# krocki/Eigen-LSTM

Measured on AMD Instinct MI355X. Metric: chars/sec fwd+BPTT, enwik6 H=512 S=100 B=64, 1/2/4/8 GPU, higher is better.
Workload: dtype f32; 1 GPU; configs[2] (headline): enwik6.txt, hidden=512 seq=100 batch=64, fp32; run as hidden=512 seq=100 batch=64/GPU (global 64), fp32, enwik6-sized synthetic text (1000000 bytes), stride-1 windows from a full window, Adagrad lr=0.01; parallelism=single, engine=default, gemm=native

## Files before the change

eigen-lstm_amd/csrc/persistent.hip:

```cpp
#include <type_traits>
#include "kernels.h"
#include "../../include/lstm_hip.h"

#include <cstdlib>

namespace lstmk {

typedef float f32x4 __attribute__((ext_vector_type(4)));
typedef unsigned int u32x4 __attribute__((ext_vector_type(4)));

#pragma clang fp contract(off)
__device__ __forceinline__ float p_exp_neg(float x) {
    const float hi = 1.44269502162933349609375f, lo = 1.925963033500011e-08f;
    const float t = -x * hi;
    const float r = __builtin_fmaf(-x, hi, -t) - x * lo;
    return __builtin_amdgcn_exp2f(t) * (1.0f + r * 0.693147180559945f);
}
template <bool FAST> __device__ __forceinline__ float p_sigm(float x) {
    if (FAST) return __frcp_rn(1.0f + __expf(-x));
    return __builtin_amdgcn_rcpf(1.0f + p_exp_neg(x));
}
template <bool FAST> __device__ __forceinline__ float p_tanh(float x) {
    if (FAST) return 1.0f - 2.0f * __frcp_rn(__expf(2.0f * x) + 1.0f);
    const float e = p_exp_neg(2.0f * __builtin_fabsf(x));
    return __builtin_copysignf((1.0f - e) * __builtin_amdgcn_rcpf(1.0f + e), x);
}

__device__ __forceinline__ float xchg_row16(float v, int l) {
    const unsigned x = __builtin_bit_cast(unsigned, v);
    const auto r = __builtin_amdgcn_permlane16_swap(x, x, false, false);
    return __builtin_bit_cast(float, (l & 16) ? r[0] : r[1]);
}
__device__ __forceinline__ float xchg_half32(float v, int l) {
    const unsigned x = __builtin_bit_cast(unsigned, v);
    const auto r = __builtin_amdgcn_permlane32_swap(x, x, false, false);
    return __builtin_bit_cast(float, (l & 32) ? r[0] : r[1]);
}

template <int CTRL> __device__ __forceinline__ float dpp_f(float v) {
    return __builtin_bit_cast(float, __builtin_amdgcn_update_dpp(0, __builtin_bit_cast(int, v), CTRL, 0xf, 0xf, false));
}

#ifndef XCD_LOCAL
#define XCD_LOCAL 1
#endif
#ifndef XCD_FORCE_LOCAL
#define XCD_FORCE_LOCAL 0
#endif
#ifndef BWD_PF
#define BWD_PF 6
#endif
#ifndef FWD_PF
#define FWD_PF 4
#endif

#ifndef CNT_STRIDE_U
#define CNT_STRIDE_U 16
#endif
constexpr int CNT_STRIDE = CNT_STRIDE_U;
#ifndef GROUP_REMAP
#define GROUP_REMAP 1
#endif
#ifndef FWD_SH
#define FWD_SH 64
#endif
#ifndef BWD_SH
#define BWD_SH 8
#endif
constexpr int CNT_SLOTS = 64;
constexpr int SPIN_LIMIT = 1 << 21;

__device__ __forceinline__ __amdgpu_buffer_rsrc_t make_rsrc(const void *p, size_t bytes) {
    const unsigned n = bytes > 0x7ffffff0ull ? 0x7ffffff0u : (unsigned)bytes;
    return __builtin_amdgcn_make_buffer_rsrc(const_cast<void *>(p), 0, (int)n, 0x00020000);
}
__device__ __forceinline__ float4 ld_sc1(__amdgpu_buffer_rsrc_t r, int byte_off) {
    const u32x4 v = __builtin_amdgcn_raw_buffer_load_b128(r, byte_off, 0, 16);
    float4 f;
    f.x = __uint_as_float(v.x);
    f.y = __uint_as_float(v.y);
    f.z = __uint_as_float(v.z);
    f.w = __uint_as_float(v.w);
    return f;
}
__device__ __forceinline__ void st_sc1(float4 f, __amdgpu_buffer_rsrc_t r, int byte_off) {
    u32x4 v;
    v.x = __float_as_uint(f.x);
    v.y = __float_as_uint(f.y);
    v.z = __float_as_uint(f.z);
    v.w = __float_as_uint(f.w);
    __builtin_amdgcn_raw_buffer_store_b128(v, r, byte_off, 0, 16);
}

#ifndef POLL_SLEEP
#define POLL_SLEEP 1
#endif
template <int CNT_SH>
__device__ __forceinline__ bool wait_arrivals(const unsigned *cp, int n_prod, unsigned epoch, unsigned *abortp, int lane) {
    const unsigned expect = lane < CNT_SH ? epoch * (unsigned)((n_prod - lane + CNT_SH - 1) / CNT_SH) : 0u;
    for (int spins = 0;; spins++) {
        unsigned v = 0;
        if (lane < CNT_SH) v = __hip_atomic_load(cp + lane * CNT_STRIDE, __ATOMIC_RELAXED, __HIP_MEMORY_SCOPE_AGENT);
        if (__all(v >= expect)) return true;
        if (spins > SPIN_LIMIT) break;
        if ((spins & 255) == 255 && __hip_atomic_load(abortp, __ATOMIC_RELAXED, __HIP_MEMORY_SCOPE_AGENT) != 0) break;
        __builtin_amdgcn_s_sleep(POLL_SLEEP);
    }
    if (lane == 0) __hip_atomic_store(abortp, 1u, __ATOMIC_RELAXED, __HIP_MEMORY_SCOPE_AGENT);
    return false;
}

template <int NK4W, bool FAST>
__global__ __launch_bounds__(256) void k_fwd_persistent(const float4 *__restrict__ Ufwd, const float *__restrict__ W,
                                                        const float *__restrict__ bias, float *H, float *__restrict__ C,
                                                        float *__restrict__ G, const int32_t *__restrict__ xi,
                                                        unsigned *cnt, unsigned *abortp, unsigned epoch, int S, int B) {
    constexpr int N = 64 * NK4W, G4 = 4 * N, nk4 = N / 16;
    __shared__ float red[4 * 4 * 64];
    __shared__ int s_abort;
    const int l = threadIdx.x & 63, w = threadIdx.x >> 6;
    const int NB = gridDim.x, NG = gridDim.y;
    const int lin_ = blockIdx.x + NB * blockIdx.y;
    const int p = GROUP_REMAP ? lin_ / NG : (int)blockIdx.x, g = GROUP_REMAP ? lin_ % NG : (int)blockIdx.y;
    const int q = l >> 4, c = l & 15;
    const int col = 16 * g + c, colc = col < B ? col : B - 1;
    const int j = 4 * p + q;

    float4 a[NK4W];
#pragma unroll
    for (int i = 0; i < NK4W; i++) a[i] = Ufwd[((size_t)p * nk4 + w * NK4W + i) * 64 + l];
    float bs[4] = {0.f, 0.f, 0.f, 0.f}, cprev = 0.f;
    if (w == 0) {
#pragma unroll
        for (int gt = 0; gt < 4; gt++) bs[gt] = bias[gt * N + j];
        cprev = C[(size_t)colc * N + j];
    }
    const __amdgpu_buffer_rsrc_t rH = make_rsrc(H, (size_t)S * N * B * sizeof(float));
    if (threadIdx.x == 0) s_abort = 0;
    __syncthreads();
    for (int t = 1; t < S; t++) {
        float wx[4] = {0.f, 0.f, 0.f, 0.f};
        if (w == 0) {
            const int x = xi[t * B + colc];
            if (x >= 0) {
#pragma unroll
                for (int gt = 0; gt < 4; gt++) wx[gt] = W[(size_t)x * G4 + gt * N + j];
            }
            if (t > 1) {
                const unsigned *cp = cnt + (size_t)((t - 1) * NG + g) * CNT_SLOTS * CNT_STRIDE;
                if (!wait_arrivals<FWD_SH>(cp, NB, epoch, abortp, l) && l == 0) s_abort = 1;
            }
        }
        __syncthreads();
        if (s_abort) return;

        const int off = (int)((((size_t)(t - 1) * B + colc) * N + 16 * (w * NK4W) + 4 * q) * sizeof(float));
        constexpr int PF = FWD_PF < NK4W ? FWD_PF : NK4W;
        float4 b[NK4W];
#pragma unroll
        for (int i = 0; i < PF; i++) b[i] = ld_sc1(rH, off + 64 * i);
        __builtin_amdgcn_sched_barrier(0);
        f32x4 acc0 = {0.f, 0.f, 0.f, 0.f}, acc1 = {0.f, 0.f, 0.f, 0.f};
#pragma unroll
        for (int i = 0; i < NK4W; i++) {
            if (i + PF < NK4W) b[i + PF] = ld_sc1(rH, off + 64 * (i + PF));
            if (i & 1) {
                acc1 = __builtin_amdgcn_mfma_f32_16x16x4f32(a[i].x, b[i].x, acc1, 0, 0, 0);
                acc1 = __builtin_amdgcn_mfma_f32_16x16x4f32(a[i].y, b[i].y, acc1, 0, 0, 0);
                acc1 = __builtin_amdgcn_mfma_f32_16x16x4f32(a[i].z, b[i].z, acc1, 0, 0, 0);
                acc1 = __builtin_amdgcn_mfma_f32_16x16x4f32(a[i].w, b[i].w, acc1, 0, 0, 0);
            } else {
                acc0 = __builtin_amdgcn_mfma_f32_16x16x4f32(a[i].x, b[i].x, acc0, 0, 0, 0);
                acc0 = __builtin_amdgcn_mfma_f32_16x16x4f32(a[i].y, b[i].y, acc0, 0, 0, 0);
                acc0 = __builtin_amdgcn_mfma_f32_16x16x4f32(a[i].z, b[i].z, acc0, 0, 0, 0);
                acc0 = __builtin_amdgcn_mfma_f32_16x16x4f32(a[i].w, b[i].w, acc0, 0, 0, 0);
            }
            __builtin_amdgcn_sched_barrier(0);
        }
#pragma unroll
        for (int r = 0; r < 4; r++) red[(w * 4 + r) * 64 + l] = acc0[r] + acc1[r];
        __syncthreads();

        if (w == 0) {
            float pre[4];
#pragma unroll
            for (int gt = 0; gt < 4; gt++) {
                const float uh = ((red[(0 * 4 + gt) * 64 + l] + red[(1 * 4 + gt) * 64 + l]) + red[(2 * 4 + gt) * 64 + l]) +
                                 red[(3 * 4 + gt) * 64 + l];
                pre[gt] = (wx[gt] + uh) + bs[gt];
            }
            const float ig = p_sigm<FAST>(pre[0]), og = p_sigm<FAST>(pre[1]), fg = p_sigm<FAST>(pre[2]);
            const float ug = p_tanh<FAST>(pre[3]);
            const float cv = p_tanh<FAST>(ig * ug + fg * cprev);
            const float hv = og * cv;
            cprev = cv;
            float4 h4;
            h4.x = __shfl(hv, c, 64);
            h4.y = __shfl(hv, 16 + c, 64);
            h4.z = __shfl(hv, 32 + c, 64);
            h4.w = __shfl(hv, 48 + c, 64);
                if (q == 0 && col < B) st_sc1(h4, rH, (int)((((size_t)t * B + col) * N + 4 * p) * sizeof(float)));
            if (t + 1 < S) {
                asm volatile("s_waitcnt vmcnt(0)" ::: "memory");
                        if (l == 0)
                    __hip_atomic_fetch_add(cnt + ((size_t)(t * NG + g) * CNT_SLOTS + (p & (FWD_SH - 1))) * CNT_STRIDE, 1u, __ATOMIC_RELAXED,
                                           __HIP_MEMORY_SCOPE_AGENT);
            }
            if (col < B) {
                float *gc = G + ((size_t)t * B + col) * G4 + j;
                gc[0] = ig;
                gc[N] = og;
                gc[2 * N] = fg;
                gc[3 * N] = ug;
                C[((size_t)t * B + col) * N + j] = cv;
            }
        }
    }
}

template <int NKW, bool FAST>
__global__ __launch_bounds__(512) void k_fwd_persistent2(const float4 *__restrict__ Ufwd, const float *__restrict__ W,
                                                         const float *__restrict__ bias, float *H, float *__restrict__ C,
                                                         float *__restrict__ G, const int32_t *__restrict__ xi,
                                                         unsigned *cnt, unsigned *abortp, unsigned epoch, int S, int B) {
    constexpr int N = 128 * NKW, G4 = 4 * N, nk4 = N / 16;
    __shared__ float red[8 * 2 * 4 * 64];
    __shared__ int s_abort;
    const int l = threadIdx.x & 63, w = threadIdx.x >> 6;
    const int NB2 = gridDim.x, NG = gridDim.y;
    const int lin_ = blockIdx.x + NB2 * blockIdx.y;
    const int p2 = GROUP_REMAP ? lin_ / NG : (int)blockIdx.x, g = GROUP_REMAP ? lin_ % NG : (int)blockIdx.y;
    const int q = l >> 4, c = l & 15;
    const int col = 16 * g + c, colc = col < B ? col : B - 1;
    const int p = 2 * p2 + (w & 1);
    const int j = 4 * p + q;

    float4 a0[NKW], a1[NKW];
#pragma unroll
    for (int i = 0; i < NKW; i++) {
        a0[i] = Ufwd[((size_t)(2 * p2) * nk4 + w * NKW + i) * 64 + l];
        a1[i] = Ufwd[((size_t)(2 * p2 + 1) * nk4 + w * NKW + i) * 64 + l];
    }
    float bs[4] = {0.f, 0.f, 0.f, 0.f}, cprev = 0.f;
    if (w < 2) {
#pragma unroll
// ... 290 lines not shown
            h4.w = dpp_f<0xFF>(hv);
            FSTAMP(8, 2)
            asm volatile("s_waitcnt vmcnt(0)" ::: "memory");
            FSTAMP(8, 3)
            if ((gu & 3) == 0 && col < B) {
                const float4 hp = {hx_canon(h4.x), hx_canon(h4.y), hx_canon(h4.z), hx_canon(h4.w)};
                const float4 sent = {__uint_as_float(HX_SENT), __uint_as_float(HX_SENT), __uint_as_float(HX_SENT),
                                     __uint_as_float(HX_SENT)};
                const size_t e_pub = ((size_t)((t + ring_base) & (HX_RING - 1)) * B + col) * N + j;
                const size_t e_rst = ((size_t)((t + 2 + ring_base) & (HX_RING - 1)) * B + col) * N + j;
                if (XCD_LOCAL && local_pub) {
                    *reinterpret_cast<float4 *>(Hx + e_pub) = hp;
                    *reinterpret_cast<float4 *>(Hx + e_rst) = sent;
                } else {
                    st_sc1(hp, rHx, (int)(e_pub * sizeof(float)));
                    st_sc1(sent, rHx, (int)(e_rst * sizeof(float)));
                }
                *reinterpret_cast<float4 *>(H + ((size_t)t * B + col) * N + j) = h4;
            }
            if (col < B) {
                float *gcp = G + ((size_t)t * B + col) * G4 + j;
                gcp[0] = ig;
                gcp[N] = og;
                gcp[2 * N] = fg;
                gcp[3 * N] = ug_;
                C[((size_t)t * B + col) * N + j] = cv;
            }
            FSTAMP(8, 4)
        }
    }
}
#undef FSTAMP
#undef FSTAMP_VAL

#define FSTAMP(wave, k)                                                                                        \
    if (STAMP && l == 0 && w == (wave) && (blockIdx.x == 0 || blockIdx.x == gridDim.x / 2) && blockIdx.y == 0) \
        stamps[((size_t)(blockIdx.x ? 1 : 0) * S + t) * 16 + (k)] = __builtin_amdgcn_s_memtime();
template <int N_, bool FAST, bool STAMP = false>
__global__ __launch_bounds__(FWD4_THREADS) void k_fwd_persistent6(const float4 *__restrict__ Ufwd5, const float *__restrict__ W,
                                                                  const float *__restrict__ bias, float *H, float *__restrict__ C,
                                                                  float *__restrict__ G, const int32_t *__restrict__ xi,
                                                                  float *Hx, unsigned *cnt, unsigned *abortp, unsigned epoch,
                                                                  int ring_base, int S, int B, int poll_cfg,
                                                                  unsigned long long *stamps = nullptr) {
    constexpr int N = N_, G4 = 4 * N, Kw = N / 8, RS = 68;
    constexpr int NAB = Kw / 4;
    static_assert(N == 512 || N == 256, "one 16-byte load per lane covers a wave's K-slice of a half (N = 256: half the lanes)");
    __shared__ __attribute__((aligned(16))) float red[2][2][8 * 4 * RS];
    __shared__ int s_abort;
    __shared__ unsigned s_done[2][2];
    const int tid = threadIdx.x, l = tid & 63, w = tid >> 6;
    const int pin_ng = (poll_cfg >> 16) & 15;
    const int g0 = (poll_cfg >> 20) & 255;
    const int GC = (poll_cfg >> 28) & 1 ? 4 : 8;
    const int NB3 = gridDim.x, NG = pin_ng ? pin_ng : (int)gridDim.y;
    const int lin_ = blockIdx.x + NB3 * blockIdx.y;
    const int kb = pin_ng ? lin_ >> 3 : GROUP_REMAP ? lin_ / NG : (int)blockIdx.x;
    const int g = pin_ng ? lin_ & 7 : GROUP_REMAP ? lin_ % NG : (int)blockIdx.y;
    if (pin_ng && g >= NG) return;
    const __amdgpu_buffer_rsrc_t rH = make_rsrc(H, (size_t)S * N * B * sizeof(float));
    const __amdgpu_buffer_rsrc_t rHx = make_rsrc(Hx, (size_t)HX_RING * N * B * sizeof(float));
    unsigned *xcc_tab = cnt + (size_t)g * CNT_SLOTS * CNT_STRIDE;
    if (tid == 0) {
        s_abort = 0;
        s_done[0][0] = s_done[0][1] = s_done[1][0] = s_done[1][1] = 0;
        if (XCD_LOCAL) {
            __hip_atomic_store(xcc_tab + kb, (epoch << 4) | (__builtin_amdgcn_s_getreg(6164) & 15u), __ATOMIC_RELAXED,
                               __HIP_MEMORY_SCOPE_AGENT);
            asm volatile("s_waitcnt vmcnt(0)" ::: "memory");
        }
    }
    const int poll_sleep = poll_cfg & 255;
    __syncthreads();

    if (w < 8) {
        const int lb = l >> 2, li = l & 3;
        const bool ld_lane = lb < NAB;
        float4 wq[NAB];
#pragma unroll
        for (int ab = 0; ab < NAB; ab++) wq[ab] = Ufwd5[(((size_t)kb * 8 + w) * NAB + ab) * 64 + l];
        int colv[2];
#pragma unroll
        for (int hf = 0; hf < 2; hf++) {
            const int c = GC * (g + g0) + 4 * hf + li;
            colv[hf] = c < B ? c : B - 1;
        }
        float4 bvq[2];
#pragma unroll
        for (int hf = 0; hf < 2; hf++)
            bvq[hf] = ld_lane ? ld_sc1(rH, (int)((((size_t)colv[hf]) * N + Kw * w + 4 * lb) * sizeof(float))) : float4{0.f, 0.f, 0.f, 0.f};
        for (int t = 1; t < S; t++) {
#pragma unroll
            for (int hf = 0; hf < 2; hf++) {
                if (hf == 1 && GC == 4) continue;
                if (hf == 0) { FSTAMP(3, 8) }
                float4 bv = bvq[hf];
                if (t > 1 && !__all(hx_ready(bv))) {
                    const int slot = (t - 1 + ring_base) & (HX_RING - 1);
                    const int off = (int)((((size_t)slot * B + colv[hf]) * N + Kw * w + 4 * lb) * sizeof(float));
                    bool ok = false;
                    for (int spins = 0; spins <= SPIN_LIMIT; spins++) {
                        bv = ld_lane ? ld_sc1(rHx, off) : float4{0.f, 0.f, 0.f, 0.f};
                        if (__all(hx_ready(bv))) {
                            ok = true;
                            break;
                        }
                        if ((spins & 255) == 255 && __hip_atomic_load(abortp, __ATOMIC_RELAXED, __HIP_MEMORY_SCOPE_AGENT) != 0) break;
                        for (int i = 0; i < poll_sleep; i++) __builtin_amdgcn_s_sleep(1);
                    }
                    if (!ok) {
                        if (l == 0) {
                            __hip_atomic_store(abortp, 1u, __ATOMIC_RELAXED, __HIP_MEMORY_SCOPE_AGENT);
                            __hip_atomic_store(&s_abort, 1, __ATOMIC_RELAXED, __HIP_MEMORY_SCOPE_WORKGROUP);
                        }
                        return;
                    }
                }
                if (hf == 0) { FSTAMP(3, 9) } else { FSTAMP(3, 5) }
                const int nslot = (t - 1 + hf + ring_base) & (HX_RING - 1);
                const int noff = (int)((((size_t)nslot * B + colv[hf ^ 1]) * N + Kw * w + 4 * lb) * sizeof(float));
                const bool req = GC == 8 && (hf == 0 ? t > 1 : t + 1 < S);
                f32x4 c0 = {0.f, 0.f, 0.f, 0.f}, c1 = c0, c2 = c0, c3 = c0;
#define F6(ab)                                                              \
    c0 = __builtin_amdgcn_mfma_f32_4x4x1f32(bv.x, wq[ab].x, c0, 4, ab, 0); \
    c1 = __builtin_amdgcn_mfma_f32_4x4x1f32(bv.y, wq[ab].y, c1, 4, ab, 0); \
    c2 = __builtin_amdgcn_mfma_f32_4x4x1f32(bv.z, wq[ab].z, c2, 4, ab, 0); \
    c3 = __builtin_amdgcn_mfma_f32_4x4x1f32(bv.w, wq[ab].w, c3, 4, ab, 0);
                F6(0) F6(1) F6(2) F6(3) F6(4) F6(5) F6(6) F6(7)
                if constexpr (NAB == 16) { F6(NAB - 8) F6(NAB - 7) F6(NAB - 6) F6(NAB - 5) F6(NAB - 4) F6(NAB - 3) F6(NAB - 2) F6(NAB - 1) }
#undef F6
                __builtin_amdgcn_sched_barrier(0);
                if (req) bvq[hf ^ 1] = ld_lane ? ld_sc1(rHx, noff) : float4{0.f, 0.f, 0.f, 0.f};
                if (GC == 4) {
                    const float sv = __uint_as_float(HX_SENT);
                    bvq[0] = ld_lane ? float4{sv, sv, sv, sv} : float4{0.f, 0.f, 0.f, 0.f};
                }
                __builtin_amdgcn_sched_barrier(0);
                if (hf == 0) { FSTAMP(3, 10) } else { FSTAMP(3, 6) }
                float *rp = red[hf][t & 1];
#pragma unroll
                for (int r = 0; r < 4; r++) rp[(w * 4 + r) * RS + l] = (c0[r] + c1[r]) + (c2[r] + c3[r]);
                asm volatile("" ::: "memory");
                if (l == 0) __hip_atomic_fetch_add(&s_done[hf][t & 1], 1u, __ATOMIC_RELAXED, __HIP_MEMORY_SCOPE_WORKGROUP);
                if (hf == 0) { FSTAMP(3, 11) } else { FSTAMP(3, 7) }
            }
        }
    } else {
        const int hf = w - 8;
        if (hf == 1 && GC == 4) return;
        __builtin_amdgcn_s_setprio(3);
        const int gc = l >> 4, gu = l & 15;
        const int col = GC * (g + g0) + 4 * hf + gc, colc = col < B ? col : B - 1;
        const int j = 16 * kb + gu;
        float bs[4], cprev, wx[4] = {0.f, 0.f, 0.f, 0.f};
#pragma unroll
        for (int gt = 0; gt < 4; gt++) bs[gt] = bias[gt * N + j];
        cprev = C[(size_t)colc * N + j];
        int xnext = xi[1 * B + colc];
        bool local_pub = false;
        const float *rp0 = red[hf][0] + gc * RS + 4 * gu;
        for (int t = 1; t < S; t++) {
#pragma unroll
            for (int gt = 0; gt < 4; gt++) wx[gt] = 0.f;
            if (xnext >= 0) {
#pragma unroll
                for (int gt = 0; gt < 4; gt++) wx[gt] = W[(size_t)xnext * G4 + gt * N + j];
            }
            if (t + 1 < S) xnext = xi[(t + 1) * B + colc];
            FSTAMP(8, 0)
            {
                bool in = false;
                for (int spins = 0; spins <= SPIN_LIMIT; spins++) {
                    in = __hip_atomic_load(&s_done[hf][t & 1], __ATOMIC_RELAXED, __HIP_MEMORY_SCOPE_WORKGROUP) >= 8u * (unsigned)((t + 1) / 2);
                    if (in || __hip_atomic_load(&s_abort, __ATOMIC_RELAXED, __HIP_MEMORY_SCOPE_WORKGROUP)) break;
                    __builtin_amdgcn_s_sleep(1);
                }
                if (!in) {
                    if (l == 0) {
                        __hip_atomic_store(abortp, 1u, __ATOMIC_RELAXED, __HIP_MEMORY_SCOPE_AGENT);
                        __hip_atomic_store(&s_abort, 1, __ATOMIC_RELAXED, __HIP_MEMORY_SCOPE_WORKGROUP);
                    }
                    return;
                }
                asm volatile("" ::: "memory");
            }
            const float *rp = rp0 + (t & 1) * (8 * 4 * RS);
            FSTAMP(8, 1)
            if (XCD_LOCAL && t == 2) {
                unsigned mine = 0;
                bool same = true;
                if (l < NB3) {
                    mine = __hip_atomic_load(xcc_tab + l, __ATOMIC_RELAXED, __HIP_MEMORY_SCOPE_AGENT);
                    same = (mine >> 4) == epoch;
                }
                const unsigned first = __builtin_amdgcn_readfirstlane(mine);
                if (l < NB3) same = same && mine == first;
                local_pub = (XCD_FORCE_LOCAL || __all(same)) && NB3 <= 64;
            }
            float4 uh = *reinterpret_cast<const float4 *>(rp);
#pragma unroll
            for (int ww = 1; ww < 8; ww++) {
                const float4 v = *reinterpret_cast<const float4 *>(rp + ww * 4 * RS);
                uh.x += v.x;
                uh.y += v.y;
                uh.z += v.z;
                uh.w += v.w;
            }
            const float pre0 = (wx[0] + uh.x) + bs[0], pre1 = (wx[1] + uh.y) + bs[1];
            const float pre2 = (wx[2] + uh.z) + bs[2], pre3 = (wx[3] + uh.w) + bs[3];
            const float ig = p_sigm<FAST>(pre0), og = p_sigm<FAST>(pre1), fg = p_sigm<FAST>(pre2);
            const float ug_ = p_tanh<FAST>(pre3);
            const float cv = p_tanh<FAST>(ig * ug_ + fg * cprev);
            const float hv = og * cv;
            cprev = cv;
            float4 h4;
            h4.x = dpp_f<0x00>(hv);
            h4.y = dpp_f<0x55>(hv);
            h4.z = dpp_f<0xAA>(hv);
            h4.w = dpp_f<0xFF>(hv);
            FSTAMP(8, 2)
            asm volatile("s_waitcnt vmcnt(0)" ::: "memory");
            FSTAMP(8, 3)
            if ((gu & 3) == 0 && col < B) {
                const float4 hp = {hx_canon(h4.x), hx_canon(h4.y), hx_canon(h4.z), hx_canon(h4.w)};
                const float4 sent = {__uint_as_float(HX_SENT), __uint_as_float(HX_SENT), __uint_as_float(HX_SENT),
                                     __uint_as_float(HX_SENT)};
                const size_t e_pub = ((size_t)((t + ring_base) & (HX_RING - 1)) * B + col) * N + j;
                const size_t e_rst = ((size_t)((t + 2 + ring_base) & (HX_RING - 1)) * B + col) * N + j;
                if (XCD_LOCAL && local_pub) {
                    *reinterpret_cast<float4 *>(Hx + e_pub) = hp;
                    *reinterpret_cast<float4 *>(Hx + e_rst) = sent;
                } else {
                    st_sc1(hp, rHx, (int)(e_pub * sizeof(float)));
                    st_sc1(sent, rHx, (int)(e_rst * sizeof(float)));
                }
                *reinterpret_cast<float4 *>(H + ((size_t)t * B + col) * N + j) = h4;
            }
            if (col < B) {
                float *gcp = G + ((size_t)t * B + col) * G4 + j;
                gcp[0] = ig;
                gcp[N] = og;
                gcp[2 * N] = fg;
                gcp[3 * N] = ug_;
                C[((size_t)t * B + col) * N + j] = cv;
            }
            FSTAMP(8, 4)
        }
    }
}
#undef FSTAMP

typedef __bf16 bf16x8 __attribute__((ext_vector_type(8)));
__device__ __forceinline__ unsigned pack_bf16x2(float lo, float hi) {
    return (unsigned)__builtin_bit_cast(unsigned short, (__bf16)lo) |
           ((unsigned)__builtin_bit_cast(unsigned short, (__bf16)hi) << 16);
}
__device__ __forceinline__ u32x4 pack_bf16x8(const float4 &a, const float4 &b) {
    u32x4 v;
    v.x = pack_bf16x2(a.x, a.y);
    v.y = pack_bf16x2(a.z, a.w);
    v.z = pack_bf16x2(b.x, b.y);
    v.w = pack_bf16x2(b.z, b.w);
    return v;
}

__global__ __launch_bounds__(256) void k_pack_U6_bf16(const float *__restrict__ U, uint2 *__restrict__ Ubwd6b, int N, int UW) {
    const int G4 = 4 * N, NS = N >= 512 ? N / 512 : 1, NPW = N / (64 * NS);
    const size_t total = (size_t)N * N;
    for (size_t e = (size_t)blockIdx.x * blockDim.x + threadIdx.x; e < total; e += (size_t)gridDim.x * blockDim.x) {
        const int l = (int)(e & 63), ab = (int)((e >> 6) % UW);
        const size_t r = (e >> 6) / UW;
        const int sx = (int)(r % NS), w = (int)((r / NS) % NPW), kb = (int)(r / ((size_t)NS * NPW));
        const int out = (w * NS + sx) * 64 + l;
        float v[4];
#pragma unroll
        for (int q = 0; q < 4; q++) {
            const int kk = 4 * ab + q, row = (kk / UW) * N + UW * kb + (kk % UW);
            v[q] = U[(size_t)out * G4 + row];
        }
        Ubwd6b[e] = uint2{pack_bf16x2(v[0], v[1]), pack_bf16x2(v[2], v[3])};
    }
}
int bwd_scatter_bf16_units(int N);
void pack_U6_bf16(const float *U, void *Ubwd6b, int N, hipStream_t st) {
    const size_t n = (size_t)N * N;
    int blocks = (int)((n + 255) / 256);
    if (blocks > 2048) blocks = 2048;
    hipLaunchKernelGGL(k_pack_U6_bf16, dim3(blocks), dim3(256), 0, st, U, reinterpret_cast<uint2 *>(Ubwd6b), N, bwd_scatter_bf16_units(N));
}
__global__ __launch_bounds__(256) void k_pack_U_bf16(const float *__restrict__ U, u32x4 *__restrict__ Ufwd16,
                                                     u32x4 *__restrict__ Ubwd16, int N) {
    const int G4 = 4 * N;
    const size_t n16 = (size_t)N * N / 2;
    for (size_t e = (size_t)blockIdx.x * blockDim.x + threadIdx.x; e < 2 * n16; e += (size_t)gridDim.x * blockDim.x) {
        float v[8];
        if (e < n16) {
            const int l = (int)(e & 63);
            const size_t qq = e >> 6;
            const int ks = (int)(qq % (N / 32)), p = (int)(qq / (N / 32));
            const int row = (l & 3) * N + 4 * p + ((l & 15) >> 2), k = 32 * ks + 8 * (l >> 4);
#pragma unroll
            for (int j = 0; j < 8; j++) v[j] = U[(size_t)(k + j) * G4 + row];
        } else {
            const size_t e2 = e - n16;
            const int l = (int)(e2 & 63);
            const size_t qq = e2 >> 6;
            const int rs = (int)(qq % (G4 / 32)), kb = (int)(qq / (G4 / 32));
            const float *src = U + (size_t)(16 * kb + (l & 15)) * G4 + 32 * rs + 8 * (l >> 4);
#pragma unroll
            for (int j = 0; j < 8; j++) v[j] = src[j];
        }
        u32x4 o;
        o.x = pack_bf16x2(v[0], v[1]);
        o.y = pack_bf16x2(v[2], v[3]);
        o.z = pack_bf16x2(v[4], v[5]);
        o.w = pack_bf16x2(v[6], v[7]);
        if (e < n16) Ufwd16[e] = o;
        else Ubwd16[e - n16] = o;
    }
}
void pack_U_bf16(const float *U, void *Ufwd16, void *Ubwd16, int N, hipStream_t st) {
    const size_t n = (size_t)N * N;
    int blocks = (int)((n + 255) / 256);
    if (blocks > 2048) blocks = 2048;
    hipLaunchKernelGGL(k_pack_U_bf16, dim3(blocks), dim3(256), 0, st, U, reinterpret_cast<u32x4 *>(Ufwd16),
                       reinterpret_cast<u32x4 *>(Ubwd16), N);
}

template <int NKS, bool FAST>
__global__ __launch_bounds__(256) void k_fwd_persistent_bf16(const u32x4 *__restrict__ Ufwd16, const float *__restrict__ W,
                                                             const float *__restrict__ bias, float *__restrict__ H,
                                                             unsigned short *Hb, float *__restrict__ C,
                                                             float *__restrict__ G, const int32_t *__restrict__ xi,
                                                             unsigned *cnt, unsigned *abortp, unsigned epoch, int S,
                                                             int B) {
    constexpr int N = 128 * NKS, G4 = 4 * N;
    __shared__ float red[4 * 4 * 64];
    __shared__ int s_abort;
    const int l = threadIdx.x & 63, w = threadIdx.x >> 6;
    const int NB = gridDim.x, NG = gridDim.y;
    const int lin_ = blockIdx.x + NB * blockIdx.y;
    const int p = GROUP_REMAP ? lin_ / NG : (int)blockIdx.x, g = GROUP_REMAP ? lin_ % NG : (int)blockIdx.y;
    const int q = l >> 4, c = l & 15;
    const int col = 16 * g + c, colc = col < B ? col : B - 1;
    const int j = 4 * p + q;

    u32x4 a[NKS];
#pragma unroll
    for (int i = 0; i < NKS; i++) a[i] = Ufwd16[((size_t)p * (N / 32) + w * NKS + i) * 64 + l];
    float bs[4] = {0.f, 0.f, 0.f, 0.f}, cprev = 0.f;
    if (w == 0) {
#pragma unroll
        for (int gt = 0; gt < 4; gt++) bs[gt] = bias[gt * N + j];
        cprev = C[(size_t)colc * N + j];
    }
    const __amdgpu_buffer_rsrc_t rHb = make_rsrc(Hb, (size_t)S * N * B * sizeof(unsigned short));
    if (threadIdx.x == 0) s_abort = 0;
    __syncthreads();

    for (int t = 1; t < S; t++) {
        float wx[4] = {0.f, 0.f, 0.f, 0.f};
        if (w == 0) {
            const int x = xi[t * B + colc];
            if (x >= 0) {
#pragma unroll
                for (int gt = 0; gt < 4; gt++) wx[gt] = W[(size_t)x * G4 + gt * N + j];
            }
            if (t > 1) {
                const unsigned *cp = cnt + (size_t)((t - 1) * NG + g) * CNT_SLOTS * CNT_STRIDE;
                if (!wait_arrivals<FWD_SH>(cp, NB, epoch, abortp, l) && l == 0) s_abort = 1;
            }
        }
        __syncthreads();
        if (s_abort) return;

        u32x4 b[NKS];
        if (t == 1) {
            const float *hp = H + (size_t)colc * N + 32 * (w * NKS) + 8 * q;
#pragma unroll
            for (int i = 0; i < NKS; i++)
                b[i] = pack_bf16x8(*reinterpret_cast<const float4 *>(hp + 32 * i), *reinterpret_cast<const float4 *>(hp + 32 * i + 4));
        } else {
            const int off = (int)((((size_t)(t - 1) * B + colc) * N + 32 * (w * NKS) + 8 * q) * sizeof(unsigned short));
#pragma unroll
            for (int i = 0; i < NKS; i++) b[i] = __builtin_amdgcn_raw_buffer_load_b128(rHb, off + 64 * i, 0, 16);
        }
        f32x4 acc = {0.f, 0.f, 0.f, 0.f};
#pragma unroll
        for (int i = 0; i < NKS; i++)
            acc = __builtin_amdgcn_mfma_f32_16x16x32_bf16(__builtin_bit_cast(bf16x8, a[i]), __builtin_bit_cast(bf16x8, b[i]), acc,
                                                          0, 0, 0);
#pragma unroll
        for (int r = 0; r < 4; r++) red[(w * 4 + r) * 64 + l] = acc[r];
        __syncthreads();

        if (w == 0) {
            float pre[4];
// ... 648 lines not shown
        float *dst = dhyb + (tu & 3) * 128;
        OL_HALF(a0, a1, a2, a3, 0);
        if (!one_half) OL_HALF(b0, b1, b2, b3, 1);
        HSTAMP(11, 14)
        if (tu >= 2) OL_REQUEST(tu - 1);
        if (FUSE && tu >= 2) h_request(tu - 1);
        OL_DROP_B();
        asm volatile("" ::: "memory");
        if (l == 0) __hip_atomic_store(s_ol, (unsigned)(S - tu), __ATOMIC_RELAXED, __HIP_MEMORY_SCOPE_WORKGROUP);
        HSTAMP(11, 15)
    }
#undef OL_DROP_B
#undef OL_HALF
#undef Y_STEP
#undef OL_REQUEST
    if (FUSE) {
        __syncthreads();
        __syncthreads();
    }
}
template <int N_, bool FUSE, bool STAMP> __device__ __forceinline__ void bwdh_weight_sums(const BwdhArgs &p) {
    BWDH_COMMON(p)
    auto xfetch = [&](int tu) -> int {
        const int col = GC_ * gq + (l & 7);
        const int x = col < B && (l & 7) < GC_ ? xi[(size_t)tu * B + col] : -2;
        return x == -1 ? 256 : x;
    };
    int xnext = xfetch(S - 1);
    for (int tu = S - 1; tu >= 1; tu--) {
        const int xcur = xnext;
        if (tu >= 2) xnext = xfetch(tu - 1);
        bool ok = true;
#pragma unroll
        for (int hf = 0; hf < 2; hf++) {
            if (hf == 1 && GC_ == 4) continue;
            if (!ok) break;
            if (!lds_wait(&s_stage[hf], (unsigned)(S - tu))) {
                ok = false;
                break;
            }
            const float *sg_ = stage + (hf * 4 + (tu & 3)) * 256;
            float sv[4];
#pragma unroll
            for (int c = 0; c < 4; c++) sv[c] = sg_[c * 64 + l];
#pragma unroll
            for (int c = 0; c < 4; c++) {
                const int x = __builtin_amdgcn_readlane(xcur, 4 * hf + c);
                if (x >= 0) dWt[x * 64 + l] += sv[c];
            }
        }
        if (!ok) {
            give_up();
            break;
        }
        asm volatile("" ::: "memory");
        if (l == 0) __hip_atomic_store(s_tab, (unsigned)(S - tu), __ATOMIC_RELAXED, __HIP_MEMORY_SCOPE_WORKGROUP);
    }
    __syncthreads();
    if (__hip_atomic_load(s_abort, __ATOMIC_RELAXED, __HIP_MEMORY_SCOPE_WORKGROUP)) return;
    table_out();
    __syncthreads();
}
#define SSTAMP(wave, k)                                                                                        \
    if (STAMP && l == 0 && w == (wave) && (blockIdx.x == 0 || blockIdx.x == gridDim.x / 2) && blockIdx.y == 0) \
        stamps[((size_t)(blockIdx.x ? 1 : 0) * S + t) * 16 + (k)] = __builtin_amdgcn_s_memtime();
__host__ __device__ inline size_t bwds_ring_floats(int N, int B) { return (size_t)HX_RING * ((B + 7) / 8) * 2 * (N / 16) * (N / 16) * 64; }

template <int N_, bool FUSE, bool STAMP> __device__ __forceinline__ void bwds_product(const BwdhArgs &p) {
    BWDH_COMMON(p)
    constexpr int NB = N / 16, NPW = N / 64;
    float *dgl = red;
    unsigned *s_loc = sync_ + 12;
    __builtin_amdgcn_s_setprio(2);
    const bool active = w < NPW;
    const int lb = l >> 2, lj = l & 3;
    float4 a[16];
#pragma unroll
    for (int ab = 0; ab < 16; ab++) a[ab] = active ? Ubwd5[(((size_t)kb * NPW + w) * 16 + ab) * 64 + l] : float4{0.f, 0.f, 0.f, 0.f};
#pragma unroll
    for (int ab = 0; ab < 16; ab++) asm volatile("" ::"v"(a[ab].x), "v"(a[ab].y), "v"(a[ab].z), "v"(a[ab].w));
    const int d = 4 * w + (lb >> 2), u = 4 * (lb & 3) + lj;
    const __amdgpu_buffer_rsrc_t rQ = make_rsrc(DGx, bwds_ring_floats(N, B) * sizeof(float));
    auto qoff = [&](int tt, int hf) {
        const size_t slot = (size_t)((tagged_ ? ring_base + (S - 1 - tt) : tt + ring_base) & (HX_RING - 1));
        return (((slot * NRG_ + rg0_ + hf) * NB + d) * NB + kb) * 64 + (size_t)u * 4;
    };
    const int wmg = w >> 1, wq0 = 2 * (w & 1);
    f32x4 wacc0 = {0.f, 0.f, 0.f, 0.f}, wacc1 = wacc0;
    float hq[8], dq[8];
    unsigned *s_wy = sync_ + 14;
    float *wyS = red + 1024;
    auto wfetch = [&](int tu) -> bool {
        if (!lds_wait(s_wy, (unsigned)(S - tu))) return false;
        const float *sp = wyS + (tu % 3) * (8 * 272);
#pragma unroll
        for (int c = 0; c < 8; c++) {
            dq[c] = sp[c * 272 + 64 * wmg + l];
            hq[c] = sp[c * 272 + 256 + (l & 15)];
        }
        return true;
    };
    auto wrelease = [&]() {
        asm volatile("" ::: "memory");
        if (l == 0) __hip_atomic_fetch_add(&sync_[15], 1u, __ATOMIC_RELAXED, __HIP_MEMORY_SCOPE_WORKGROUP);
    };
    auto wstep = [&]() {
#pragma unroll
        for (int c = 0; c < 8; c++) {
            if (wq0 == 0) {
                wacc0 = __builtin_amdgcn_mfma_f32_4x4x1f32(hq[c], dq[c], wacc0, 4, 0, 0);
                wacc1 = __builtin_amdgcn_mfma_f32_4x4x1f32(hq[c], dq[c], wacc1, 4, 1, 0);
            } else {
                wacc0 = __builtin_amdgcn_mfma_f32_4x4x1f32(hq[c], dq[c], wacc0, 4, 2, 0);
                wacc1 = __builtin_amdgcn_mfma_f32_4x4x1f32(hq[c], dq[c], wacc1, 4, 3, 0);
            }
        }
    };
    bool live = true;
    for (int t = S - 1; t >= 2 && live; t--) {
#pragma unroll
        for (int hf = 0; hf < 2; hf++) {
            if (hf == 1 && GC_ == 4) continue;
            if (!live) break;
            if (hf == 0) { SSTAMP(3, 8) }
            if (!lds_wait(&s_done[2 * hf + (t & 1)], (unsigned)((S - 1 - t) / 2 + 1))) {
                give_up();
                live = false;
                break;
            }
            if (hf == 0) { SSTAMP(3, 9) } else { SSTAMP(3, 5) }
            if (active) {
                const float4 dv = *reinterpret_cast<const float4 *>(dgl + (hf * 2 + (t & 1)) * 256 + lj * 64 + 4 * lb);
                const bool local = t < S - 1 && __hip_atomic_load(&s_loc[hf], __ATOMIC_RELAXED, __HIP_MEMORY_SCOPE_WORKGROUP) != 0;
                f32x4 c0 = {0.f, 0.f, 0.f, 0.f}, c1 = c0, c2 = c0, c3 = c0;
#define S6(ab)                                                            \
    c0 = __builtin_amdgcn_mfma_f32_4x4x1f32(dv.x, a[ab].x, c0, 4, ab, 0); \
    c1 = __builtin_amdgcn_mfma_f32_4x4x1f32(dv.y, a[ab].y, c1, 4, ab, 0); \
    c2 = __builtin_amdgcn_mfma_f32_4x4x1f32(dv.z, a[ab].z, c2, 4, ab, 0); \
    c3 = __builtin_amdgcn_mfma_f32_4x4x1f32(dv.w, a[ab].w, c3, 4, ab, 0);
                S6(0) S6(1) S6(2) S6(3) S6(4) S6(5) S6(6) S6(7) S6(8) S6(9) S6(10) S6(11) S6(12) S6(13) S6(14) S6(15)
#undef S6
                if (hf == 0) { SSTAMP(3, 10) } else { SSTAMP(3, 6) }
                float4 q;
                q.x = hx_canon((c0[0] + c1[0]) + (c2[0] + c3[0]));
                q.y = hx_canon((c0[1] + c1[1]) + (c2[1] + c3[1]));
                q.z = hx_canon((c0[2] + c1[2]) + (c2[2] + c3[2]));
                q.w = hx_canon((c0[3] + c1[3]) + (c2[3] + c3[3]));
                if (tagged_) {
                    const unsigned ph = (unsigned)((ring_base + (S - 1 - t)) >> 2) & 1u;
                    q = float4{tag_mark(q.x, ph), tag_mark(q.y, ph), tag_mark(q.z, ph), tag_mark(q.w, ph)};
                }
                const float4 sent = {__uint_as_float(HX_SENT), __uint_as_float(HX_SENT), __uint_as_float(HX_SENT),
                                     __uint_as_float(HX_SENT)};
                asm volatile("s_waitcnt vmcnt(0)" ::: "memory");
                const size_t e_pub = qoff(t, hf), e_rst = qoff(t - 2, hf);
                if (d < NB) {
                    if (XCD_LOCAL && local) {
                        *reinterpret_cast<float4 *>(DGx + e_pub) = q;
                        if (!tagged_) *reinterpret_cast<float4 *>(DGx + e_rst) = sent;
                    } else {
                        st_sc1(q, rQ, (int)(e_pub * sizeof(float)));
                        if (!tagged_) st_sc1(sent, rQ, (int)(e_rst * sizeof(float)));
                    }
                }
                if (hf == 0) { SSTAMP(3, 11) } else { SSTAMP(3, 7) }
            }
        }
        if (FUSE && live) {
            if (!wfetch(t)) {
                give_up();
                live = false;
                break;
            }
            if (!(cfg & 8)) wstep();
            wrelease();
        }
    }
    if (FUSE && live) {
        if (wfetch(1)) {
            if (!(cfg & 8)) wstep();
            wrelease();
        } else
            give_up();
    }
    if (FUSE) {
        __syncthreads();
        if (__hip_atomic_load(s_abort, __ATOMIC_RELAXED, __HIP_MEMORY_SCOPE_WORKGROUP)) return;
        {
            float *Yp = base + (size_t)G4 * 256 + (size_t)G4 * N + G4 + (size_t)(16 * kb) * 256 + 64 * wmg + l;
#pragma unroll
            for (int i = 0; i < 4; i++) {
                Yp[(size_t)(4 * wq0 + i) * 256] = wacc0[i];
                Yp[(size_t)(4 * (wq0 + 1) + i) * 256] = wacc1[i];
            }
        }
        table_out();
        __syncthreads();
        if (w == 0) {
            const int gt = l >> 4, rj = l & 15;
            float sum = 0.0f;
            for (int c = 0; c < 8; c++) sum += dbs[(c * 4 + gt) * 16 + rj];
            base[(size_t)G4 * 256 + (size_t)G4 * N + gt * N + 16 * kb + rj] = sum;
        }
    }
}
template <int N_, bool FUSE, bool STAMP> __device__ __forceinline__ void bwds_elementwise(const BwdhArgs &p) {
    BWDH_COMMON(p)
    constexpr int NB = N / 16, NLD = NB / 4;
    float *dgl = red;
    unsigned *s_loc = sync_ + 12;
    const int hf = w - 8;
    __builtin_amdgcn_s_setprio(3);
    const int cc = l >> 4, jj = l & 15;
    const int ecol = GC_ * gq + 4 * hf + cc, ecolc = ecol < B ? ecol : B - 1;
    const int j = 16 * kb + jj;
    float dcn = 0.0f;
    bool local_pub = false;
    float dbacc[4] = {0.f, 0.f, 0.f, 0.f};
    const __amdgpu_buffer_rsrc_t rQ = make_rsrc(DGx, bwds_ring_floats(N, B) * sizeof(float));
    auto qbase = [&](int tt) {
        const size_t slot = (size_t)((tagged_ ? ring_base + (S - 1 - tt) : tt + ring_base) & (HX_RING - 1));
        return (int)(((((slot * NRG_ + rg0_ + hf) * NB + kb) * NB + (size_t)(l >> 4)) * 64 + (size_t)(l & 15) * 4) * sizeof(float));
    };
    float ig, og, fg, ug, cv, cp;
    auto fetch = [&](int tu) {
        const float *gc = G + ((size_t)tu * B + ecolc) * G4 + j;
        ig = gc[0], og = gc[N], fg = gc[2 * N], ug = gc[3 * N];
        cv = C[((size_t)tu * B + ecolc) * N + j], cp = C[((size_t)(tu - 1) * B + ecolc) * N + j];
    };
    fetch(S - 1);
    float dhy = 0.0f;
    const bool alive = lds_wait(s_ol, 1u);
    if (alive) dhy = dhyb[((S - 1) & 3) * 128 + (4 * hf + cc) * 16 + jj];
    else give_up();
    const bool idle = hf == 1 && GC_ == 4;
    for (int t = S - 1; t >= 1 && alive && !idle; t--) {
        SSTAMP(8, 0)
        float dhn = 0.0f;
        if (t < S - 1) {
            const int off = qbase(t + 1);
            const unsigned ph = (unsigned)((ring_base + (S - 2 - t)) >> 2) & 1u;
            float4 v[NLD];
            bool ok = false;
            for (int spins = 0; spins <= SPIN_LIMIT; spins++) {
                bool gd = true;
#pragma unroll
                for (int i = 0; i < NLD; i++) v[i] = ld_sc1(rQ, off + i * (4 * 64 * (int)sizeof(float)));
#pragma unroll
                for (int i = 0; i < NLD; i++) gd = gd && (tagged_ ? tag_ready(v[i], ph) : hx_ready(v[i]));
                if (__all(gd)) {
                    ok = true;
                    break;
                }
                if ((spins & 255) == 255 && __hip_atomic_load(abortp, __ATOMIC_RELAXED, __HIP_MEMORY_SCOPE_AGENT) != 0) break;
                for (int i = 0; i < ((cfg >> 9) & 7); i++) __builtin_amdgcn_s_sleep(1);
            }
            if (!ok) {
                give_up();
                break;
            }
            SSTAMP(8, 1)
            if (tagged_) {
#pragma unroll
                for (int i = 0; i < NLD; i++) v[i] = float4{tag_value(v[i].x), tag_value(v[i].y), tag_value(v[i].z), tag_value(v[i].w)};
            }
            float4 sm = v[0];
#pragma unroll
            for (int i = 1; i < NLD; i++) {
                sm.x += v[i].x;
                sm.y += v[i].y;
                sm.z += v[i].z;
                sm.w += v[i].w;
            }
            const int q = l >> 4;
            const float k0 = (q & 1) ? sm.y : sm.x, k1 = (q & 1) ? sm.w : sm.z;
            const float s0 = (q & 1) ? sm.x : sm.y, s1 = (q & 1) ? sm.z : sm.w;
            const float z0 = k0 + xchg_row16(s0, l), z1 = k1 + xchg_row16(s1, l);
            const float keep = (q & 2) ? z1 : z0, send = (q & 2) ? z0 : z1;
            dhn = keep + xchg_half32(send, l);
        }
        if (XCD_LOCAL && t == S - 2) {
            unsigned mine = 0;
            bool same = true;
            if (l < NBK) {
                mine = __hip_atomic_load(xcc_tab + l, __ATOMIC_RELAXED, __HIP_MEMORY_SCOPE_AGENT);
                same = (mine >> 4) == epoch;
            }
            const unsigned first = __builtin_amdgcn_readfirstlane(mine);
            if (l < NBK) same = same && mine == first;
            local_pub = (XCD_FORCE_LOCAL || __all(same)) && NBK <= 64;
            if (l == 0) __hip_atomic_store(&s_loc[hf], local_pub ? 1u : 0u, __ATOMIC_RELAXED, __HIP_MEMORY_SCOPE_WORKGROUP);
        }
        const float dh = dhy + dhn;
        float dcv = dh * og + dcn;
        dcv = dcv * (1.0f - cv * cv);
        const float d_o = (dh * cv) * (og * (1.0f - og));
        const float d_i = (dcv * ug) * (ig * (1.0f - ig));
        const float d_f = (dcv * cp) * (fg * (1.0f - fg));
        const float d_u = (dcv * ig) * (1.0f - ug * ug);
        dcn = dcv * fg;
        SSTAMP(8, 2)
        {
            float *dp = dgl + (hf * 2 + (t & 1)) * 256 + cc * 64 + jj;
            dp[0] = d_i;
            dp[16] = d_o;
            dp[32] = d_f;
            dp[48] = d_u;
            asm volatile("" ::: "memory");
            if (l == 0) __hip_atomic_fetch_add(&s_done[2 * hf + (t & 1)], 1u, __ATOMIC_RELAXED, __HIP_MEMORY_SCOPE_WORKGROUP);
        }
        SSTAMP(8, 3)
        const int ta = jj & 3, tq = jj >> 2;
        float t0 = d_i, t1 = d_o, t2 = d_f, t3 = d_u;
        {
            const float lo = (ta & 1) ? t0 : t1, hi = (ta & 1) ? t2 : t3;
            const float rlo = dpp_f<0xB1>(lo), rhi = dpp_f<0xB1>(hi);
// ... 1462 lines not shown
```

Measured before the change: 9.716 million chars/s.

## Prefetch embedding rows a step ahead and relax vmcnt waits in persistent LSTM

```diff
diff --git a/eigen-lstm_amd/csrc/persistent.hip b/eigen-lstm_amd/csrc/persistent.hip
--- a/eigen-lstm_amd/csrc/persistent.hip
+++ b/eigen-lstm_amd/csrc/persistent.hip
@@ -91,6 +91,19 @@
     v.w = __float_as_uint(f.w);
     __builtin_amdgcn_raw_buffer_store_b128(v, r, byte_off, 0, 16);
 }
+constexpr int BUF_DROP = 0x7ffffff0;
+__device__ __forceinline__ void st_buf(float4 f, __amdgpu_buffer_rsrc_t r, int byte_off) {
+    u32x4 v;
+    v.x = __float_as_uint(f.x);
+    v.y = __float_as_uint(f.y);
+    v.z = __float_as_uint(f.z);
+    v.w = __float_as_uint(f.w);
+    __builtin_amdgcn_raw_buffer_store_b128(v, r, byte_off, 0, 0);
+}
+__device__ __forceinline__ void st_buf(float f, __amdgpu_buffer_rsrc_t r, int byte_off) {
+    __builtin_amdgcn_raw_buffer_store_b32(__float_as_uint(f), r, byte_off, 0, 0);
+}
+#define WAIT_VMCNT(n) __builtin_amdgcn_s_waitcnt(0x0F70 | ((n) & 15) | (((n) >> 4) << 14))
 
 #ifndef POLL_SLEEP
 #define POLL_SLEEP 1
@@ -687,21 +700,26 @@
         const int gc = l >> 4, gu = l & 15;
         const int col = GC * (g + g0) + 4 * hf + gc, colc = col < B ? col : B - 1;
         const int j = 16 * kb + gu;
-        float bs[4], cprev, wx[4] = {0.f, 0.f, 0.f, 0.f};
+        float bs[4], cprev, wr[4];
 #pragma unroll
         for (int gt = 0; gt < 4; gt++) bs[gt] = bias[gt * N + j];
         cprev = C[(size_t)colc * N + j];
         int xnext = xi[1 * B + colc];
+        bool xok;
+        auto wgather = [&]() {
+            xok = xnext >= 0;
+            const int xs = xok ? xnext : 0;
+#pragma unroll
+            for (int gt = 0; gt < 4; gt++) wr[gt] = W[(size_t)xs * G4 + gt * N + j];
+        };
+        wgather();
+        xnext = xi[(S > 2 ? 2 : 1) * B + colc];
+        asm volatile("" ::"v"(bs[0]), "v"(bs[1]), "v"(bs[2]), "v"(bs[3]), "v"(cprev), "v"(wr[0]), "v"(wr[1]), "v"(wr[2]),
+                     "v"(wr[3]), "v"(xnext));
         bool local_pub = false;
         const float *rp0 = red[hf][0] + gc * RS + 4 * gu;
+        const bool pub_lane = (gu & 3) == 0 && col < B;
         for (int t = 1; t < S; t++) {
-#pragma unroll
-            for (int gt = 0; gt < 4; gt++) wx[gt] = 0.f;
-            if (xnext >= 0) {
-#pragma unroll
-                for (int gt = 0; gt < 4; gt++) wx[gt] = W[(size_t)xnext * G4 + gt * N + j];
-            }
-            if (t + 1 < S) xnext = xi[(t + 1) * B + colc];
             FSTAMP(8, 0)
             {
                 bool in = false;
@@ -741,8 +759,9 @@
                 uh.z += v.z;
                 uh.w += v.w;
             }
-            const float pre0 = (wx[0] + uh.x) + bs[0], pre1 = (wx[1] + uh.y) + bs[1];
-            const float pre2 = (wx[2] + uh.z) + bs[2], pre3 = (wx[3] + uh.w) + bs[3];
+            const float wx0 = xok ? wr[0] : 0.f, wx1 = xok ? wr[1] : 0.f, wx2 = xok ? wr[2] : 0.f, wx3 = xok ? wr[3] : 0.f;
+            const float pre0 = (wx0 + uh.x) + bs[0], pre1 = (wx1 + uh.y) + bs[1];
+            const float pre2 = (wx2 + uh.z) + bs[2], pre3 = (wx3 + uh.w) + bs[3];
             const float ig = p_sigm<FAST>(pre0), og = p_sigm<FAST>(pre1), fg = p_sigm<FAST>(pre2);
             const float ug_ = p_tanh<FAST>(pre3);
             const float cv = p_tanh<FAST>(ig * ug_ + fg * cprev);
@@ -754,30 +773,35 @@
             h4.z = dpp_f<0xAA>(hv);
             h4.w = dpp_f<0xFF>(hv);
             FSTAMP(8, 2)
-            asm volatile("s_waitcnt vmcnt(0)" ::: "memory");
+            WAIT_VMCNT(11);
             FSTAMP(8, 3)
-            if ((gu & 3) == 0 && col < B) {
+            {
                 const float4 hp = {hx_canon(h4.x), hx_canon(h4.y), hx_canon(h4.z), hx_canon(h4.w)};
                 const float4 sent = {__uint_as_float(HX_SENT), __uint_as_float(HX_SENT), __uint_as_float(HX_SENT),
                                      __uint_as_float(HX_SENT)};
-                const size_t e_pub = ((size_t)((t + ring_base) & (HX_RING - 1)) * B + col) * N + j;
-                const size_t e_rst = ((size_t)((t + 2 + ring_base) & (HX_RING - 1)) * B + col) * N + j;
+                const int o_pub = pub_lane ? (int)(((((size_t)((t + ring_base) & (HX_RING - 1)) * B + col) * N + j) * sizeof(float))) : BUF_DROP;
+                const int o_rst = pub_lane ? (int)(((((size_t)((t + 2 + ring_base) & (HX_RING - 1)) * B + col) * N + j) * sizeof(float))) : BUF_DROP;
                 if (XCD_LOCAL && local_pub) {
-                    *reinterpret_cast<float4 *>(Hx + e_pub) = hp;
-                    *reinterpret_cast<float4 *>(Hx + e_rst) = sent;
+                    st_buf(hp, rHx, o_pub);
+                    st_buf(sent, rHx, o_rst);
                 } else {
-                    st_sc1(hp, rHx, (int)(e_pub * sizeof(float)));
-                    st_sc1(sent, rHx, (int)(e_rst * sizeof(float)));
-                }
-                *reinterpret_cast<float4 *>(H + ((size_t)t * B + col) * N + j) = h4;
-            }
-            if (col < B) {
-                float *gcp = G + ((size_t)t * B + col) * G4 + j;
-                gcp[0] = ig;
-                gcp[N] = og;
-                gcp[2 * N] = fg;
-                gcp[3 * N] = ug_;
-                C[((size_t)t * B + col) * N + j] = cv;
+                    st_sc1(hp, rHx, o_pub);
+                    st_sc1(sent, rHx, o_rst);
+                }
+            }
+            wgather();
+            xnext = xi[(t + 2 < S ? t + 2 : S - 1) * B + colc];
+            {
+                const __amdgpu_buffer_rsrc_t rHt = make_rsrc(H + (size_t)t * B * N, (size_t)B * N * sizeof(float));
+                const __amdgpu_buffer_rsrc_t rCt = make_rsrc(C + (size_t)t * B * N, (size_t)B * N * sizeof(float));
+                const __amdgpu_buffer_rsrc_t rGt = make_rsrc(G + (size_t)t * B * G4, (size_t)B * G4 * sizeof(float));
+                st_buf(h4, rHt, pub_lane ? (int)(((size_t)col * N + j) * sizeof(float)) : BUF_DROP);
+                auto og_ = [&](int gt) { return col < B ? (int)(((size_t)col * G4 + gt * N + j) * sizeof(float)) : BUF_DROP; };
+                st_buf(ig, rGt, og_(0));
+                st_buf(og, rGt, og_(1));
+                st_buf(fg, rGt, og_(2));
+                st_buf(ug_, rGt, og_(3));
+                st_buf(cv, rCt, col < B ? (int)(((size_t)col * N + j) * sizeof(float)) : BUF_DROP);
             }
             FSTAMP(8, 4)
         }
@@ -1732,16 +1756,15 @@
                 }
                 const float4 sent = {__uint_as_float(HX_SENT), __uint_as_float(HX_SENT), __uint_as_float(HX_SENT),
                                      __uint_as_float(HX_SENT)};
-                asm volatile("s_waitcnt vmcnt(0)" ::: "memory");
+                if (tagged_ || GC_ == 4) asm volatile("s_waitcnt vmcnt(0)" ::: "memory");
+                else asm volatile("s_waitcnt vmcnt(2)" ::: "memory");
                 const size_t e_pub = qoff(t, hf), e_rst = qoff(t - 2, hf);
-                if (d < NB) {
-                    if (XCD_LOCAL && local) {
-                        *reinterpret_cast<float4 *>(DGx + e_pub) = q;
-                        if (!tagged_) *reinterpret_cast<float4 *>(DGx + e_rst) = sent;
-                    } else {
-                        st_sc1(q, rQ, (int)(e_pub * sizeof(float)));
-                        if (!tagged_) st_sc1(sent, rQ, (int)(e_rst * sizeof(float)));
-                    }
+                if (XCD_LOCAL && local) {
+                    *reinterpret_cast<float4 *>(DGx + e_pub) = q;
+                    if (!tagged_) *reinterpret_cast<float4 *>(DGx + e_rst) = sent;
+                } else {
+                    st_sc1(q, rQ, (int)(e_pub * sizeof(float)));
+                    if (!tagged_) st_sc1(sent, rQ, (int)(e_rst * sizeof(float)));
                 }
                 if (hf == 0) { SSTAMP(3, 11) } else { SSTAMP(3, 7) }
             }
```

Result: no change. 9.785 million chars/s, median of 6 (+0.7%).
